# 10XGenomics/supernova

Measured on AMD Instinct MI355X. Metric: Gk-mers/s through count+graph at k=48, 1.2B×150bp; bit-exact counts, higher is better.
Workload: dtype u64

## Files before the change

supernova_amd/csrc/snk_count.hip:

```cpp
#include "snk_ctx.h"
#include "snk_common.h"
#include "snk_kernels.h"
#include "snk_stages.h"

namespace {

constexpr uint32_t BC_MULTI = 0xFFFFFFFEu;
constexpr uint32_t BC_IGN = 0xFFFFFFFFu;
static_assert(BC_IGN > BC_MULTI, "barcode states are merged with atomicMax");
#ifndef SNK_TIGHT_TRIES
#define SNK_TIGHT_TRIES 48
#endif
constexpr int MAX_SPLIT_LOG2 = 20;
#define SNK_COUNT_MAXSEG 32
#ifndef SNK_COUNT_THREADS
#define SNK_COUNT_THREADS 768
#endif
#ifndef SNK_SCREEN_ROUNDS
#define SNK_SCREEN_ROUNDS 6
#endif
#ifndef SNK_GSCREEN_SLOTS
#define SNK_GSCREEN_SLOTS 1024
#endif
#ifndef SNK_GSCREEN_BATCH
#define SNK_GSCREEN_BATCH 512
#endif
#ifndef SNK_GSCREEN_ROUNDS
#define SNK_GSCREEN_ROUNDS (SNK_SCREEN_ROUNDS + 4)
#endif
#ifndef SNK_NGSCREEN_PLANE_WORDS
#define SNK_NGSCREEN_PLANE_WORDS 512
#endif
#ifndef SNK_COUNT_SLOTS
#define SNK_COUNT_SLOTS 2048
#endif
#define LDS_LOAD(p) __hip_atomic_load((p), __ATOMIC_RELAXED, __HIP_MEMORY_SCOPE_WORKGROUP)
__device__ __forceinline__ void lds_barrier() { asm volatile("s_waitcnt lgkmcnt(0)\n\ts_barrier" ::: "memory"); }
#ifdef SNK_COUNT_PROF
#define PROF(n) do { if (tid == 0) { const long long _t = clock64(); prof_acc[n] += (unsigned long long)(_t - prof_t); prof_t = _t; } } while (0)
#else
#define PROF(n) do {} while (0)
#endif

__device__ __forceinline__ uint32_t funnel(uint32_t hi, uint32_t lo, uint32_t sh) {
#ifdef SNK_FUNNEL_ALIGNBIT
    return sh ? __builtin_amdgcn_alignbit(hi, lo, 32u - sh) : hi;
#else
    return (uint32_t)(((((uint64_t)hi << 32) | lo) << sh) >> 32);
#endif
}

template <int K> struct lo_t { typedef uint32_t type; };
template <> struct lo_t<60> { typedef uint64_t type; };

template <int K> __device__ __forceinline__ typename lo_t<K>::type lo_pack(uint64_t lo);
template <> __device__ __forceinline__ uint32_t lo_pack<48>(uint64_t lo) { return (uint32_t)(lo >> 32); }
template <> __device__ __forceinline__ uint64_t lo_pack<60>(uint64_t lo) { return lo; }
template <int K> __device__ __forceinline__ uint64_t lo_unpack(typename lo_t<K>::type v);
template <> __device__ __forceinline__ uint64_t lo_unpack<48>(uint32_t v) { return (uint64_t)v << 32; }
template <> __device__ __forceinline__ uint64_t lo_unpack<60>(uint64_t v) { return v; }

template <int K, bool G> struct klo_t { typedef typename lo_t<K>::type type; };
template <int K> struct klo_t<K, true> { typedef uint64_t type; };
template <int K, bool G> __device__ __forceinline__ typename klo_t<K, G>::type klo_pack(uint64_t lo) {
    if constexpr (G) return lo; else return lo_pack<K>(lo);
}
template <int K, bool G> __device__ __forceinline__ uint64_t klo_unpack(typename klo_t<K, G>::type v) {
    if constexpr (G) return v; else return lo_unpack<K>(v);
}

typedef __attribute__((address_space(3))) void* snk_lptr;

template <int K, int THREADS, int SLOTS, bool GROUPED, bool MULTI, bool GATHER = false, bool TIGHT = false, bool SCREEN = false>
__global__ void __launch_bounds__(THREADS, 6) snk_count_kernel(snk_count_args a) {
    constexpr int BATCH = (GROUPED && SCREEN && SLOTS <= 1024 && K == 48) ? SNK_GSCREEN_BATCH : ((K == 48 && !GROUPED && (SLOTS >= 2048 || SCREEN)) ? 512 : 256);
    constexpr int DD = 2 * BATCH;
    typedef typename klo_t<K, GROUPED>::type lo_type;
    constexpr int WMAX = K - SNK_M_MIN_OF(K) + 1;
    constexpr int NCI = BATCH * WMAX / 32 + 2;
    extern __shared__ __attribute__((aligned(16))) unsigned char smem_raw[];
    uint64_t* khi = reinterpret_cast<uint64_t*>(smem_raw);
    lo_type* klo = reinterpret_cast<lo_type*>(khi + SLOTS);
    uint32_t* tag = reinterpret_cast<uint32_t*>(klo + SLOTS);
    uint32_t* cnt = tag + SLOTS;
    uint32_t* bcs = cnt + SLOTS;
    uint32_t* ctxw = bcs + SLOTS;
    uint32_t* rec = ctxw + SLOTS / 4;
    uint32_t* ctl = rec + 8 * BATCH;
    uint32_t* dd = ctl + (TIGHT ? 72 : 64);
    uint32_t* wgt = dd + DD;
    uint16_t* lead = reinterpret_cast<uint16_t*>(wgt + BATCH);
    uint16_t* lpre = lead + BATCH;
    uint16_t* cidx = lpre + BATCH + 2;
    uint32_t* segi = reinterpret_cast<uint32_t*>(smem_raw + (((size_t)(reinterpret_cast<unsigned char*>(cidx + NCI) - smem_raw) + 15) & ~(size_t)15));
    uint16_t* olist = reinterpret_cast<uint16_t*>(segi + 2 * 3 * SNK_COUNT_MAXSEG);
    uint32_t* bcx = reinterpret_cast<uint32_t*>(smem_raw + (((size_t)(reinterpret_cast<unsigned char*>(olist + (TIGHT ? SLOTS - 64 : SLOTS - THREADS - 64)) - smem_raw) + 15) & ~(size_t)15));
    const bool bcset = a.bc_mode > 2;
    constexpr int SROUNDS = (SCREEN && SLOTS <= 1024) ? SNK_GSCREEN_ROUNDS : SNK_SCREEN_ROUNDS;
    static_assert(SROUNDS >= 1 && SROUNDS <= 16, "two cells per register");
    constexpr int SPW = GROUPED ? ((DD + BATCH) / 3 >= 512 ? 512 : 256) : SNK_NGSCREEN_PLANE_WORDS;
    constexpr uint32_t SCB = SPW == 1024 ? 17u : (SPW == 512 ? 18u : 19u);
    constexpr uint32_t SCAND = GROUPED ? (SLOTS <= 1024 ? 2048 : 1024) : 4096;
    uint16_t* cand = reinterpret_cast<uint16_t*>(bcx);
    uint32_t* planes = GROUPED ? dd : reinterpret_cast<uint32_t*>(cand + SCAND);
    static_assert(!SCREEN || (GROUPED && 3 * SPW <= DD + BATCH) || (!GROUPED && K == 48 && SLOTS <= 1024), "no room for the screen's bit planes");
    static_assert(THREADS >= BATCH && THREADS % 64 == 0, "the first BATCH threads own the staged records");
    const int tid = threadIdx.x;
    const int lane = tid & 63;
    const uint32_t LIMIT = TIGHT ? min(a.tight & 0xFFFFu, (uint32_t)SLOTS - 64u) : SLOTS - THREADS - 64;
    const int tight_tries = (int)(a.tight >> 16);
#ifdef SNK_COUNT_PROF
    long long prof_t = clock64();
    unsigned long long prof_acc[8] = {0, 0, 0, 0, 0, 0, 0, 0};
#endif
    auto dma_batch = [&](uint64_t base, uint64_t vend, const uint32_t* bnd, const uint32_t* seg) {
        constexpr int CH = 2 * BATCH;
        uint32_t seg_incl = 0;
        if (MULTI) {
            const uint32_t mylen = (uint32_t)lane < a.nseg ? LDS_LOAD(&seg[2 * SNK_COUNT_MAXSEG + lane]) - LDS_LOAD(&seg[lane]) : 0u;
            seg_incl = snk_wave_scan_incl(mylen);
        }
        constexpr int NR = (CH + THREADS - 1) / THREADS;
        uint32_t gx[NR];
        if (GATHER) {
#pragma unroll
            for (int r = 0; r < NR; ++r) {
                const int c = r * THREADS + tid;
                const uint64_t v = base + (uint32_t)(c >> 1);
                gx[r] = (c < CH && v < vend) ? a.gidx[v] : 0u;
            }
        }
#pragma unroll
        for (int r = 0; r * THREADS < CH; ++r) {
            const int c = r * THREADS + tid;
            const uint64_t v = base + (uint32_t)(c >> 1);
            if (c < CH && v < vend) {
                uint64_t gi;
                if (GATHER) gi = gx[r];
                else if (MULTI) {
                    const uint32_t x = (uint32_t)v;
                    uint32_t acc = 0, sg = 0;
                    for (uint32_t q = 0; q + 1 < a.nseg; ++q) { const uint32_t e = __builtin_amdgcn_readlane(seg_incl, q); if (x >= e) { sg = q + 1; acc = e; } }
                    gi = (((uint64_t)seg[SNK_COUNT_MAXSEG + sg] << 32) | seg[sg]) + (x - acc);
                } else gi = v;
                (void)bnd;
                const uint32_t lds_at = __builtin_amdgcn_readfirstlane((uint32_t)(size_t)(snk_lptr)(rec + 4 * (r * THREADS + (tid & ~63))));
                asm volatile("s_mov_b32 m0, %0\n\ts_nop 0\n\tglobal_load_lds_dwordx4 %1, off" :: "s"(lds_at), "v"(a.records + gi * 2 + (uint32_t)(c & 1)) : "memory");
            }
        }
    };
    auto bucket_range = [&](const uint32_t* bnd, const uint32_t* seg, uint64_t& vbeg, uint64_t& vend) {
        if (MULTI) {
            const uint32_t mylen = (uint32_t)lane < a.nseg ? LDS_LOAD(&seg[2 * SNK_COUNT_MAXSEG + lane]) - LDS_LOAD(&seg[lane]) : 0u;
            vbeg = 0;
            vend = (uint32_t)__builtin_amdgcn_readlane((int)snk_wave_scan_incl(mylen), 63);
        }
        else {
            vbeg = ((uint64_t)LDS_LOAD(&bnd[1]) << 32) | LDS_LOAD(&bnd[0]);
            vend = ((uint64_t)LDS_LOAD(&bnd[3]) << 32) | LDS_LOAD(&bnd[2]);
        }
    };
    const uint32_t G = a.bucket_stride;
    unsigned long long rcur = a.region_cursor[blockIdx.x];
    uint32_t bucket = a.bucket0 + (blockIdx.x + G - a.bucket0 % G) % G;
    uint32_t par = 0;
    {
        uint64_t b0 = 0, e0 = 0;
        if (tid == 0) {
            if (bucket < a.NB) { b0 = a.seg_beg[bucket]; e0 = a.seg_end[bucket]; }
            ctl[4] = (uint32_t)b0; ctl[5] = (uint32_t)(b0 >> 32); ctl[6] = (uint32_t)e0; ctl[7] = (uint32_t)(e0 >> 32);
            ctl[3] = 0;
            ctl[1] = 0; ctl[2] = 0; ctl[8] = 0; ctl[9] = 0; ctl[10] = 0; ctl[11] = 0; ctl[0] = 0;
            if (TIGHT) { ctl[64] = 0; ctl[65] = 0; }
        }
        for (int s = tid; s < SLOTS; s += THREADS) tag[s] = 0;
        if (MULTI && tid < (int)a.nseg) {
            uint64_t b = 0, e = 0;
            if (bucket < a.NB) { b = a.seg_beg[(uint64_t)tid * a.seg_stride + bucket]; e = a.seg_end[(uint64_t)tid * a.seg_stride + bucket]; }
            segi[tid] = (uint32_t)b; segi[SNK_COUNT_MAXSEG + tid] = (uint32_t)(b >> 32); segi[2 * SNK_COUNT_MAXSEG + tid] = (uint32_t)e;
        }
        lds_barrier();
        uint64_t vb, ve;
        bucket_range(ctl + 4, segi, vb, ve);
        dma_batch(vb, ve, ctl + 4, segi);
    }
    bool prefetched = true;
    uint32_t q = 0, bq = 0;
    unsigned long long claims_sum = 0;
    for (; bucket < a.NB; bucket += G) {
    uint32_t sp = 1;
    bool fresh = true;
    uint32_t splits_done = 0;
    const uint32_t nbucket = bucket + G;
    bool seg_pending = true;
    const uint32_t* bcur = ctl + 4 + 8 * par;
    uint32_t* bnext = ctl + 4 + 8 * (par ^ 1u);
    const uint32_t* segc = segi + par * (3 * SNK_COUNT_MAXSEG);
    uint32_t* segn = segi + (par ^ 1u) * (3 * SNK_COUNT_MAXSEG);
    const uint32_t sseg = MULTI ? min((uint32_t)tid, a.nseg - 1u) : 0u;
    auto load_next = [&](uint64_t& nbeg, uint64_t& nend, uint64_t& nsb, uint32_t& nse) {
        nbeg = 0; nend = 0; nsb = 0; nse = 0;
        if (nbucket < a.NB) {
            nbeg = a.seg_beg[nbucket]; nend = a.seg_end[nbucket];
            if (MULTI) { nsb = a.seg_beg[(uint64_t)sseg * a.seg_stride + nbucket]; nse = (uint32_t)a.seg_end[(uint64_t)sseg * a.seg_stride + nbucket]; }
        }
    };
    auto put_down = [&](uint64_t nbeg, uint64_t nend, uint64_t nsb, uint32_t nse) {
        bnext[0] = (uint32_t)nbeg; bnext[1] = (uint32_t)(nbeg >> 32); bnext[2] = (uint32_t)nend; bnext[3] = (uint32_t)(nend >> 32);
        if (MULTI) { segn[sseg] = (uint32_t)nsb; segn[SNK_COUNT_MAXSEG + sseg] = (uint32_t)(nsb >> 32); segn[2 * SNK_COUNT_MAXSEG + sseg] = nse; }
        seg_pending = false;
    };
    uint32_t lg0 = 0, id0 = 0, real_bucket = bucket;
    if (a.vmeta) {
        const uint2 vm = a.vmeta[bucket];
        real_bucket = __builtin_amdgcn_readfirstlane(vm.x);
        lg0 = __builtin_amdgcn_readfirstlane(vm.y >> 24);
        id0 = __builtin_amdgcn_readfirstlane(vm.y & 0xFFFFFFu);
    }
    while (sp) {
        PROF(0);
        --sp;
        uint32_t split_lg = lg0, split_id = id0;
        if (!fresh) {
            lds_barrier();
            split_lg = LDS_LOAD(&ctl[16 + 2 * sp]); split_id = LDS_LOAD(&ctl[17 + 2 * sp]);
        }
        fresh = false;
        const uint32_t split_mask = (1u << split_lg) - 1u;
        uint32_t* occ = ctl + 1 + q;
        uint32_t* place = ctl + 8 + q;
        uint32_t* resv = ctl + 64 + q;
        uint64_t vbeg, vend;
        bucket_range(bcur, segc, vbeg, vend);
        if (vbeg >= vend) {
            lds_barrier();
            if (tid == 0) { ctl[1 + (q ^ 1u)] = 0; ctl[8 + (q ^ 1u)] = 0; if (TIGHT) ctl[64 + (q ^ 1u)] = 0; }
            if (seg_pending) {
                uint64_t nbeg, nend, nsb; uint32_t nse;
                load_next(nbeg, nend, nsb, nse);
                put_down(nbeg, nend, nsb, nse);
            }
            lds_barrier();
        }
        PROF(1);
        {
            for (uint64_t base = vbeg; base < vend; base += BATCH) {
                if (!prefetched) dma_batch(base, vend, bcur, segc);
                prefetched = false;
                if (tid < BATCH) wgt[tid] = (SCREEN && GROUPED) ? 0u : 1u;
                if (SCREEN && !GROUPED) { for (int qq = tid; qq < 3 * SPW; qq += THREADS) planes[qq] = 0; }
                for (int q = tid; q < DD; q += THREADS) dd[q] = 0;
                asm volatile("s_waitcnt vmcnt(0)" ::: "memory");
                lds_barrier();
                PROF(2);
                if (tid == 0) { ctl[1 + (q ^ 1u)] = 0; ctl[8 + (q ^ 1u)] = 0; ctl[10 + (bq ^ 1u)] = 0; if (TIGHT) ctl[64 + (q ^ 1u)] = 0; if (SCREEN) ctl[0] = 0; }
                const bool fetch_next = seg_pending;
                uint64_t nbeg = 0, nend = 0, nsb = 0; uint32_t nse = 0;
                if (fetch_next) load_next(nbeg, nend, nsb, nse);
                uint32_t nkm = 0;
                if (tid < BATCH && base + tid < vend) {
                    const uint4 ra = *reinterpret_cast<const uint4*>(rec + 8 * tid), rb = *reinterpret_cast<const uint4*>(rec + 8 * tid + 4);
                    nkm = rb.z & 0x7Fu;
                    if (a.dbg == 5 && ((rb.z >> 7) & 3u) != 3u) nkm = 0;
                    if (!GROUPED && a.dbg != 4 && nkm) {
                        uint32_t h = (ra.x * 0x9E3779B1u) ^ snk_rotl32(ra.y * 0x85EBCA77u, 7) ^ (ra.z * 0xC2B2AE3Du) ^ snk_rotl32(ra.w * 0x27D4EB2Fu, 13)
                                   ^ (rb.x * 0x165667B1u) ^ snk_rotl32(rb.y * 0xcc9e2d51u, 19) ^ (rb.z * 0x1b873593u);
                        h ^= h >> 15; h *= 0x846ca68bu; h ^= h >> 13;
                        uint32_t s = h & (DD - 1);
                        for (;;) {
                            uint32_t v = LDS_LOAD(&dd[s]);
                            if (v == 0) {
                                v = atomicCAS(&dd[s], 0u, (uint32_t)tid + 1u);
                                if (v == 0) break;
                            }
                            const uint32_t L = v - 1u;
                            const uint4 la = *reinterpret_cast<const uint4*>(rec + 8 * L);
                            const uint32_t lb0 = rec[8 * L + 4], lb1 = rec[8 * L + 5], lb2 = rec[8 * L + 6];
                            bool same = ((la.x ^ ra.x) | (la.y ^ ra.y) | (la.z ^ ra.z) | (la.w ^ ra.w) | (lb0 ^ rb.x) | (lb1 ^ rb.y) | (lb2 ^ rb.z)) == 0;
                            if (GROUPED || bcset) same = same && LDS_LOAD(&rec[8 * L + 7]) == rb.w;
                            if (same) {
                                atomicAdd(&wgt[L], 1u);
                                const uint32_t mine = GROUPED ? 0u : rb.w;
                                if (mine >= BC_MULTI) atomicMax(&rec[8 * L + 7], mine);
                                else if (mine) {
                                    uint32_t ob = atomicCAS(&rec[8 * L + 7], 0u, mine);
                                    if (ob != 0 && ob != mine && ob < BC_MULTI) atomicMax(&rec[8 * L + 7], BC_MULTI);
                                }
                                nkm = 0;
                                break;
                            }
                            s = (s + 1) & (DD - 1);
                        }
                    }
                }
                const uint32_t sv = nkm | (nkm ? 0x10000u : 0u);
                uint32_t incl = sv;
                incl = snk_wave_scan_incl(incl);
// ... 90 lines not shown
                        const uint32_t m6 = rp[6], w7 = rp[7];
                        const uint32_t wt = (SCREEN && GROUPED) ? 1u : wgt[i];
                        const uint32_t n_i = m6 & 0x7Fu, hasL = (m6 >> 7) & 1u, hasR = (m6 >> 8) & 1u;
                        const uint32_t j = g + n_i - lend;
                        const uint32_t bst = GROUPED ? 0u : w7;
                        const uint32_t o = hasL + j;
                        const uint32_t wi = o >> 4, sh = (2u * o) & 31u;
                        const uint32_t* wp = rp + wi;
                        const uint32_t P = wp[-1], W0 = wp[0], W1 = wp[1], W2 = wp[2], W3 = wp[3];
                        const uint32_t F0 = funnel(W0, W1, sh), F1 = funnel(W1, W2, sh), F2 = funnel(W2, W3, sh);
                        const uint32_t pb = funnel(P, W0, sh) & 3u;
                        uint32_t F3 = 0, nb;
                        if constexpr (K == 48) nb = (W3 >> (30u - sh)) & 3u;
                        else {
                            static_assert(K == 60, "K is 48 or 60");
                            const uint32_t W4 = wp[4];
                            const uint32_t f3 = funnel(W3, W4, sh);
                            nb = (f3 >> 6) & 3u;
                            F3 = f3 & 0xFFFFFF00u;
                        }
                        const uint32_t havesucc = hasR | ((j + 1u - n_i) >> 31), havepred = min(o, 1u);
                        snk_kmer f;
                        f.hi = ((uint64_t)F0 << 32) | F1;
                        f.lo = ((uint64_t)F2 << 32) | F3;
                        const snk_kmer r = snk_kmer_rc<K>(f);
                        const bool rev = snk_kmer_lt(r, f);
                        snk_kmer c = rev ? r : f;
                        const uint32_t cfw = (havepred << (4u + pb)) | (havesucc << nb);
                        const uint32_t crv = (havesucc << (7u - nb)) | (havepred << (3u - pb));
                        const uint32_t ctx = rev ? crv : cfw;
                        if (GROUPED) c.lo |= (uint64_t)w7;
                        uint32_t h1, h2;
                        snk_kmer_hash_count<(K > 48) || GROUPED>(c, &h1, &h2);
                        if (a.dbg == 1) { if (h1 == 0x12345u && h2 == 0x54321u) a.status[3] = 7; }
                        else if ((h2 & split_mask) == split_id) {
                            uint32_t slot = h1 & (SLOTS - 1);
                            const uint32_t stride = ((h1 >> 16) ^ (h2 >> 20)) | 1u;
                            const lo_type clo = klo_pack<K, GROUPED>(c.lo);
                            const uint32_t mytag = (h2 & ~1u) | 2u;
                            bool claimed = false;
                            bool go = true;
                            uint32_t need = 0;
                            int rl = 0;
                            if constexpr (TIGHT) {
                                const unsigned long long pm = __ballot(1);
                                rl = __ffsll((long long)pm) - 1;
                                need = (uint32_t)__popcll(pm);
                                uint32_t r = 0;
                                if (lane == rl) {
                                    r = atomicAdd(resv, need);
                                    if ((r & 0x7FFFFFFFu) + need > LIMIT && !(r >> 31)) {
                                        atomicSub(resv, need);
                                        r = 0x80000000u;
                                        for (int tries = 0; tries < tight_tries; ++tries) {
                                            if (LDS_LOAD(occ) + need > LIMIT) break;
                                            const uint32_t rv = LDS_LOAD(resv);
                                            if (rv >> 31) break;
                                            if (rv + need <= LIMIT) {
                                                const uint32_t r2 = atomicAdd(resv, need);
                                                if (r2 >> 31) break;
                                                if (r2 + need <= LIMIT) { r = r2; break; }
                                                atomicSub(resv, need);
                                            }
                                            __builtin_amdgcn_s_sleep(2);
                                        }
                                        if (r >> 31) atomicOr(resv, 0x80000000u);
                                    }
                                }
                                go = (__shfl(r, rl) >> 31) == 0u;
                            }
                            if (go) {
                            for (;;) {
                                uint32_t t;
                                for (;;) {
                                    t = __hip_atomic_load(&tag[slot], __ATOMIC_ACQUIRE, __HIP_MEMORY_SCOPE_WORKGROUP);
                                    if (t == 0 || ((t ^ mytag) & ~1u) == 0) break;
                                    slot = (slot + stride) & (SLOTS - 1);
                                }
                                if (t == 0) {
                                    t = atomicCAS(&tag[slot], 0u, mytag);
                                    if (t == 0) {
                                        khi[slot] = c.hi;
                                        klo[slot] = clo;
                                        cnt[slot] = a.dbg == 2 ? 0u : wt;
                                        bcs[slot] = bst;
                                        reinterpret_cast<uint8_t*>(ctxw)[slot] = (uint8_t)ctx;
                                        if (bcset) {
#pragma unroll
                                            for (int q = 0; q < 6; ++q) bcx[slot * 6 + q] = 0;
                                        }
                                        __hip_atomic_store(&tag[slot], mytag | 1u, __ATOMIC_RELEASE, __HIP_MEMORY_SCOPE_WORKGROUP);
                                        claimed = true;
                                        break;
                                    }
                                    if (((t ^ mytag) & ~1u) != 0) { slot = (slot + stride) & (SLOTS - 1); continue; }
                                }
                                if (!(t & 1u)) continue;
                                if (khi[slot] == c.hi && klo[slot] == clo) break;
                                slot = (slot + stride) & (SLOTS - 1);
                            }
                            if constexpr (TIGHT) {
                                const uint32_t nc = (uint32_t)__popcll(__ballot(claimed));
                                if (lane == rl && need > nc) atomicSub(resv, need - nc);
                            }
                            if (claimed) {
                                const unsigned long long cm = __ballot(1);
                                const int leader = __ffsll((long long)cm) - 1;
                                uint32_t base = 0;
                                if (lane == leader) base = atomicAdd(occ, (uint32_t)__popcll(cm));
                                const uint32_t at = __shfl(base, leader) + (uint32_t)__popcll(cm & ((1ull << lane) - 1ull));
                                if (at < LIMIT) olist[at] = (uint16_t)slot;
                            } else if (a.dbg != 2) {
                                atomicAdd(&cnt[slot], wt);
                                if (ctx) atomicOr(&ctxw[slot >> 2], ctx << (8 * (slot & 3)));
                                if (bst >= BC_MULTI) atomicMax(&bcs[slot], bst);
                                else if (bst) {
                                    uint32_t ob = atomicCAS(&bcs[slot], 0u, bst);
                                    if (ob != 0 && ob != bst && ob < BC_MULTI) {
                                        if (!bcset) atomicMax(&bcs[slot], BC_MULTI);
                                        else {
                                            bool stored = false;
                                            for (int q = 0; q < 6 && !stored; ++q) {
                                                const uint32_t ov = atomicCAS(&bcx[slot * 6 + q], 0u, bst);
                                                stored = ov == 0u || ov == bst;
                                            }
                                            if (!stored) atomicMax(&bcs[slot], BC_MULTI);
                                        }
                                    }
                                }
                            }
                            }
                        }
                    }
                }
                lds_barrier();
                PROF(5);
                bq ^= 1u;
            }
        }
        if (TIGHT ? (LDS_LOAD(resv) >> 31) != 0u : LDS_LOAD(occ) > LIMIT) {
            if (split_lg >= MAX_SPLIT_LOG2) { if (tid == 0) atomicExch(&a.status[1], 1u); }
            else {
                if (tid == 0) {
                    ctl[16 + 2 * sp] = split_lg + 1; ctl[17 + 2 * sp] = split_id;
                    ctl[18 + 2 * sp] = split_lg + 1; ctl[19 + 2 * sp] = split_id | (1u << split_lg);
                }
                sp += 2;
            }
            for (int s = tid; s < SLOTS; s += THREADS) tag[s] = 0;
            ++splits_done;
            q ^= 1u;
            continue;
        }
        PROF(6);
        if (sp == 0) {
            uint64_t nvb, nve;
            bucket_range(bnext, segn, nvb, nve);
            dma_batch(nvb, nve, bnext, segn);
            prefetched = true;
        }
        const uint32_t nocc = LDS_LOAD(occ);
        const uint64_t rbase = rcur;
        const uint64_t gbase = (uint64_t)blockIdx.x * a.region_cap + rbase;
        for (uint32_t e0 = 0; e0 < nocc; e0 += THREADS) {
            const uint32_t e = e0 + tid;
            uint32_t s = 0, c = 0;
            bool ok = false;
            if (e < nocc) {
                s = olist[e];
                c = cnt[s];
                tag[s] = 0;
                ok = c >= a.min_freq && c != 0;
                if (ok && a.bc_mode) {
                    const uint32_t b = bcs[s];
                    if (!bcset) ok = a.bc_mode == 1 ? (b != 0) : (b >= BC_MULTI);
                    else {
                        uint32_t distinct = b ? 1u : 0u;
                        for (int j = 0; j < 6; ++j) distinct += bcx[s * 6 + j] ? 1u : 0u;
                        ok = b >= BC_MULTI || distinct >= a.bc_mode;
                    }
                }
            }
            const unsigned long long m = __ballot(ok);
            if (m) {
                const int leader = __ffsll((long long)m) - 1;
                uint32_t b = 0;
                if (lane == leader) b = atomicAdd(place, (uint32_t)__popcll(m));
                b = __builtin_amdgcn_readlane(b, leader);
                const uint64_t pos = rbase + b + (uint32_t)__popcll(m & ((1ull << lane) - 1ull));
                if (ok && pos < a.region_cap) {
                    const uint64_t at = gbase - rbase + pos;
                    const uint32_t cx = (ctxw[s >> 2] >> (8 * (s & 3))) & 0xFFu;
                    a.out_keys[at] = ((snk_u128)khi[s] << 64) | (snk_u128)klo_unpack<K, GROUPED>(klo[s]);
                    a.out_vals[at] = ((uint64_t)(c < 0xFFFFFFu ? c : 0xFFFFFFu) << 8) | cx;
                }
            }
        }
        lds_barrier();
        const uint32_t nvalid = LDS_LOAD(place);
        if constexpr (TIGHT) {
            if (a.chunk_n && nvalid > SNK_GRAPH_CHUNK_MAX && split_lg >= MAX_SPLIT_LOG2) { if (tid == 0) atomicExch(&a.status[1], 1u); }
            else if (a.chunk_n && nvalid > SNK_GRAPH_CHUNK_MAX) {
                if (tid == 0) {
                    ctl[16 + 2 * sp] = split_lg + 1; ctl[17 + 2 * sp] = split_id;
                    ctl[18 + 2 * sp] = split_lg + 1; ctl[19 + 2 * sp] = split_id | (1u << split_lg);
                }
                sp += 2;
                ++splits_done;
                asm volatile("s_waitcnt vmcnt(0)" ::: "memory");
                prefetched = false;
                q ^= 1u;
                continue;
            }
        }
        if (nvalid) {
            rcur += nvalid;
            if (tid == 0) {
                if (rbase + nvalid > a.region_cap) a.status[0] = 1;
                else if (a.chunk_n) {
                    if (split_lg == 0) { a.chunk_n[bucket] = nvalid; a.chunk_base[bucket] = (uint32_t)rbase; }
                    else {
                        const uint32_t e = atomicAdd(&a.status[4], 1u);
                        if (e < a.extra_cap) a.extra[e] = make_uint4(real_bucket, (uint32_t)rbase, nvalid | (blockIdx.x << 12), (split_lg << 24) | split_id);
                    }
                }
            }
        }
        claims_sum += nocc;
        if (tid == 0 && nocc > ctl[3]) ctl[3] = nocc;
        q ^= 1u;
        PROF(7);
    }
    if (tid == 0 && splits_done) atomicAdd(&a.status[2], 1u);
    par ^= 1u;
    }
    if (tid == 0) { a.region_cursor[blockIdx.x] = rcur; atomicMax(&a.status[3], ctl[3]); atomicAdd(&a.status[5], (uint32_t)(claims_sum >> 4)); }
    asm volatile("s_waitcnt vmcnt(0)" ::: "memory");
#ifdef SNK_COUNT_PROF
    if (tid == 0) for (int q = 0; q < 8; ++q) atomicAdd(&a.prof[q], prof_acc[q]);
#endif
}

template <int K> struct cfg;
template <> struct cfg<48> { static constexpr int THREADS = SNK_COUNT_THREADS; static constexpr int SLOTS = SNK_COUNT_SLOTS; };
template <> struct cfg<60> { static constexpr int THREADS = SNK_COUNT_THREADS; static constexpr int SLOTS = SNK_COUNT_SLOTS; };

template <int K, bool G>
size_t lds_bytes(uint32_t bc_mode = 0, bool tight = false, bool screen = false) {
    const size_t S = screen ? SNK_GSCREEN_SLOTS : cfg<K>::SLOTS, B = (G && screen && S <= 1024 && K == 48) ? SNK_GSCREEN_BATCH : ((K == 48 && !G && (S >= 2048 || screen)) ? 512 : 256), DD = 2 * B, NCI = B * (K - SNK_M_MIN_OF(K) + 1) / 32 + 2;
    return S * (8 + sizeof(typename klo_t<K, G>::type) + 4 + 4 + 4) + S + 4 * (8 * B + (tight ? 72 : 64) + DD + B) + 2 * (B + B + 2 + NCI) + 16 + 2 * 4 * 3 * SNK_COUNT_MAXSEG + 2 * (tight ? S - 64 : S - cfg<K>::THREADS - 64) + 16 + (bc_mode > 2 ? S * 24 + 16 : 0) + (screen ? (G ? (S <= 1024 ? 4096 : 2048) : 8192 + 3 * SNK_NGSCREEN_PLANE_WORDS * 4) + 16 : 0);
}

template <int K, bool G>
int launch(hipStream_t st, const snk_count_args& a, char* err, size_t errcap) {
    auto kern = a.nseg > 1 ? snk_count_kernel<K, cfg<K>::THREADS, cfg<K>::SLOTS, G, true> : snk_count_kernel<K, cfg<K>::THREADS, cfg<K>::SLOTS, G, false>;
    if (a.gidx) {
        if (a.nseg != 1) return snk_fail(SNK_E_INTERNAL, err, errcap, "count: an index list comes with one segment per bucket");
        kern = snk_count_kernel<K, cfg<K>::THREADS, cfg<K>::SLOTS, G, false, true>;
    }
    const bool tight = a.tight && !a.gidx;
    const bool screen = K == 48 && tight && a.screen >= 2u && a.bc_mode <= 2u;
    static_assert(SNK_GSCREEN_SLOTS <= 1024, "the ungrouped SCREEN instantiation needs the LDS half a table frees");
    if constexpr (K == 48) {
        if (screen) kern = a.nseg > 1 ? snk_count_kernel<K, cfg<K>::THREADS, SNK_GSCREEN_SLOTS, G, true, false, true, true> : snk_count_kernel<K, cfg<K>::THREADS, SNK_GSCREEN_SLOTS, G, false, false, true, true>;
    }
    if (tight && !screen) kern = a.nseg > 1 ? snk_count_kernel<K, cfg<K>::THREADS, cfg<K>::SLOTS, G, true, false, true> : snk_count_kernel<K, cfg<K>::THREADS, cfg<K>::SLOTS, G, false, false, true>;
    size_t lds = lds_bytes<K, G>(a.bc_mode, tight, screen);
    SNK_HIP_TRY(hipFuncSetAttribute((const void*)kern, hipFuncAttributeMaxDynamicSharedMemorySize, (int)lds));
    if (a.bucket0 >= a.NB) return SNK_OK;
    snk_count_args b = a;
    b.bucket_stride = a.n_regions;
    SNK_HIP_TRY(snk_launch(kern, a.n_regions, cfg<K>::THREADS, lds, st, b));
    return SNK_OK;
}

template <int K, bool G>
int regions(uint32_t nseg, uint32_t NB, uint32_t bc_mode, uint32_t persist, uint32_t* out, char* err, size_t errcap) {
    auto kern = nseg > 1 ? snk_count_kernel<K, cfg<K>::THREADS, cfg<K>::SLOTS, G, true> : snk_count_kernel<K, cfg<K>::THREADS, cfg<K>::SLOTS, G, false>;
    size_t lds = lds_bytes<K, G>(bc_mode);
    SNK_HIP_TRY(hipFuncSetAttribute((const void*)kern, hipFuncAttributeMaxDynamicSharedMemorySize, (int)lds));
    if (persist == 0) persist = 1;
    int per_cu = 0, dev = 0, n_cu = 256;
    SNK_HIP_TRY(hipOccupancyMaxActiveBlocksPerMultiprocessor(&per_cu, kern, cfg<K>::THREADS, lds));
    SNK_HIP_TRY(hipGetDevice(&dev));
    SNK_HIP_TRY(hipDeviceGetAttribute(&n_cu, hipDeviceAttributeMultiprocessorCount, dev));
    uint64_t grid = (uint64_t)(per_cu > 0 ? per_cu : 1) * (uint64_t)n_cu * persist;
    if (grid > NB) grid = NB;
    if (grid > (1u << 20)) grid = 1u << 20;
    *out = grid ? (uint32_t)grid : 1u;
    return SNK_OK;
}

}

namespace {
__global__ void __launch_bounds__(256) compact_regions_kernel(const snk_u128* __restrict__ keys_in, const uint64_t* __restrict__ vals_in,
                                                              uint64_t region_cap, const unsigned long long* __restrict__ cursor,
                                                              const unsigned long long* __restrict__ off,
                                                              snk_u128* __restrict__ keys_out, uint64_t* __restrict__ vals_out) {
    const uint32_t r = blockIdx.x;
    const uint64_t n = cursor[r], src = (uint64_t)r * region_cap, dst = off[r];
    for (uint64_t i = threadIdx.x; i < n; i += 256) {
        keys_out[dst + i] = keys_in[src + i];
        vals_out[dst + i] = vals_in[src + i];
    }
}
}

int snk_launch_compact_regions(hipStream_t st, const snk_u128* keys_in, const uint64_t* vals_in, uint64_t region_cap,
                               uint32_t n_regions, const unsigned long long* region_cursor,
                               const unsigned long long* region_off, snk_u128* keys_out, uint64_t* vals_out, char* err,
// ... 33 lines not shown
```

supernova_amd/csrc/snk_stages.hip:

```cpp
#include <string.h>
#include <cstring>
#include <rocprim/rocprim.hpp>

#include <stdlib.h>
#include <math.h>

#include <cmath>
#include <vector>

#include "snk_ctx.h"
#include "snk_common.h"
#include "snk_graph.h"
#include "snk_kernels.h"
#include "snk_stages.h"


int snk_stage_count_table(snk_ctx* ctx, hipStream_t st, uint32_t K, const void* records, const uint64_t* seg_beg,
                          const uint64_t* seg_end, uint32_t seg_stride, uint32_t nseg, uint32_t NB, uint32_t min_freq, uint32_t bc_mode, uint32_t grouped, uint64_t n_inst_hint,
                          uint32_t* status, bool want_sort, snk_table* out, char* err, size_t errcap, const snk_count_ranges* ranges, snk_count_pilot* pilot,
                          const uint32_t* gidx, bool defer_compact, const snk_hot* hot) {
    if (hot && hot->NBv == 0) hot = nullptr;
    defer_compact = defer_compact && !want_sort && snk_opt_u32(ctx, SNK_OPT_defer_compact) != 0;
    int rc;
    snk_phase_timer tm(st), kt(st);
// ... 162 lines not shown
            snk_count_args cv = ca;
            cv.records = (const uint4*)hot->records;
            cv.seg_beg = hot->seg;
            cv.seg_end = hot->seg + hot->NBv;
            cv.seg_stride = hot->NBv;
            cv.nseg = 1;
            cv.gidx = nullptr;
            cv.vmeta = hot->vmeta;
            cv.NB = hot->NBv;
            cv.bucket0 = 0;
            if ((rc = snk_launch_count(K, st, cv, err, errcap))) return rc;
        }
        if (pilot_regrow) {
            snk_ctx_release_block(ctx, keys_r);
            snk_ctx_release_block(ctx, vals_r);
            if (extra) snk_ctx_release_block(ctx, extra);
            pilot_regrown = true;
            --attempt;
            continue;
        }
        SNK_HIP_TRY(hipMemcpyAsync(h_rcur.data(), rcur, n_regions * 8ull, hipMemcpyDeviceToHost, st));
        SNK_HIP_TRY(hipMemcpyAsync(h_status, status, 32, hipMemcpyDeviceToHost, st));
        SNK_HIP_TRY(snk_sync(st));
#ifdef SNK_COUNT_PROF
        {
            unsigned long long hp[8];
            (void)hipMemcpy(hp, ca.prof, 64, hipMemcpyDeviceToHost);
            unsigned long long tot = 0;
            for (int q = 0; q < 8; ++q) tot += hp[q];
            fprintf(stderr, "[snk prof] count kernel, cycles of thread 0 per phase (%% of total): control %.1f, clear %.1f, stage %.1f, dedupe+scan %.1f, map %.1f, insert %.1f, emit-count %.1f, emit-write %.1f\n",
                    100.0 * hp[0] / tot, 100.0 * hp[1] / tot, 100.0 * hp[2] / tot, 100.0 * hp[3] / tot, 100.0 * hp[4] / tot, 100.0 * hp[5] / tot, 100.0 * hp[6] / tot, 100.0 * hp[7] / tot);
        }
#endif
        if (ca.dbg >= 2) {
            unsigned long long d[3];
            (void)hipMemcpy(d, status + 4, 24, hipMemcpyDeviceToHost);
            fprintf(stderr, "[snk dbg] lane probe iterations %llu, wave-level iterations %llu, max lane iterations in one probe %llu\n", d[0], d[1], d[2]);
        }
        if (h_status[1]) return snk_fail(SNK_E_INTERNAL, err, errcap, h_status[1] == 2 ? "count: a table probe did not terminate" : "count: bucket split depth exceeded");
        unsigned long long mx = 0;
        n_kmers = 0;
        for (uint32_t r = 0; r < n_regions; ++r) { n_kmers += h_rcur[r]; if (h_rcur[r] > mx) mx = h_rcur[r]; }
        const bool extra_ovf = !want_sort && h_status[4] > extra_cap;
        if (!h_status[0] && mx <= region_cap && !extra_ovf) break;
        if (attempt == 3) return snk_fail(SNK_E_INTERNAL, err, errcap, "count: region overflow (%llu > %llu)", mx, (unsigned long long)region_cap);
        snk_ctx_release_block(ctx, keys_r);
        snk_ctx_release_block(ctx, vals_r);
        if (mx > region_cap) region_cap = mx + 64;
        if (extra_ovf) extra_cap = h_status[4] + 64;
    }
    if (ranges && ranges->finished) ranges->finished(ranges->user);
    {
        std::vector<unsigned long long>& h_off = ctx->h_region_off;
        h_off.resize(n_regions + 1);
        unsigned long long acc = 0;
        for (uint32_t r = 0; r < n_regions; ++r) { h_off[r] = acc; acc += h_rcur[r]; }
        h_off[n_regions] = acc;
        SNK_HIP_TRY(hipMemcpyAsync(roff, h_off.data(), (n_regions + 1) * 8ull, hipMemcpyHostToDevice, st));
        void* q;
        if ((rc = snk_ctx_alloc(ctx, (n_kmers + 1) * 16, &q, err, errcap))) return rc; keys_a = (snk_u128*)q;
        if ((rc = snk_ctx_alloc(ctx, (n_kmers + 1) * 8, &q, err, errcap))) return rc; vals_a = (uint64_t*)q;
        out->keys_r = nullptr; out->vals_r = nullptr; out->region_cap = region_cap;
        if (defer_compact) {
            snk_ctx_release_block(ctx, vals_a);
            vals_a = nullptr;
            out->keys_r = keys_r; out->vals_r = vals_r;
        } else {
            if ((rc = snk_launch_compact_regions(st, keys_r, vals_r, region_cap, n_regions, rcur, roff, keys_a, vals_a, err, errcap))) return rc;
            snk_ctx_release_block(ctx, keys_r);
            snk_ctx_release_block(ctx, vals_r);
        }
// ... 764 lines not shown
```

Measured before the change: 98.21.

## Cut count-kernel SGPR pressure: cold kernarg loads, templated barcode mode, multi-segment fast path

Result: faster. 99.80 (median of 6 runs) (+1.6%).

```diff
diff --git a/supernova_amd/csrc/snk_count.hip b/supernova_amd/csrc/snk_count.hip
--- a/supernova_amd/csrc/snk_count.hip
+++ b/supernova_amd/csrc/snk_count.hip
@@ -50,6 +50,13 @@
 #endif
 }
 
+typedef const __attribute__((address_space(4))) snk_count_args* count_kargs_t;
+__device__ __forceinline__ count_kargs_t cold_args() {
+    count_kargs_t p = (count_kargs_t)__builtin_amdgcn_kernarg_segment_ptr();
+    asm volatile("" : "+s"(p));
+    return p;
+}
+
 template <int K> struct lo_t { typedef uint32_t type; };
 template <> struct lo_t<60> { typedef uint64_t type; };
 
@@ -71,7 +78,7 @@
 
 typedef __attribute__((address_space(3))) void* snk_lptr;
 
-template <int K, int THREADS, int SLOTS, bool GROUPED, bool MULTI, bool GATHER = false, bool TIGHT = false, bool SCREEN = false>
+template <int K, int THREADS, int SLOTS, bool GROUPED, bool MULTI, bool GATHER = false, bool TIGHT = false, bool SCREEN = false, bool BCSET = false>
 __global__ void __launch_bounds__(THREADS, 6) snk_count_kernel(snk_count_args a) {
     constexpr int BATCH = (GROUPED && SCREEN && SLOTS <= 1024 && K == 48) ? SNK_GSCREEN_BATCH : ((K == 48 && !GROUPED && (SLOTS >= 2048 || SCREEN)) ? 512 : 256);
     constexpr int DD = 2 * BATCH;
@@ -93,9 +100,16 @@
     uint16_t* lpre = lead + BATCH;
     uint16_t* cidx = lpre + BATCH + 2;
     uint32_t* segi = reinterpret_cast<uint32_t*>(smem_raw + (((size_t)(reinterpret_cast<unsigned char*>(cidx + NCI) - smem_raw) + 15) & ~(size_t)15));
-    uint16_t* olist = reinterpret_cast<uint16_t*>(segi + 2 * 3 * SNK_COUNT_MAXSEG);
+    uint32_t* mseg = segi + 2 * 3 * SNK_COUNT_MAXSEG;
+    uint16_t* olist = reinterpret_cast<uint16_t*>(mseg + 4);
     uint32_t* bcx = reinterpret_cast<uint32_t*>(smem_raw + (((size_t)(reinterpret_cast<unsigned char*>(olist + (TIGHT ? SLOTS - 64 : SLOTS - THREADS - 64)) - smem_raw) + 15) & ~(size_t)15));
-    const bool bcset = a.bc_mode > 2;
+    constexpr bool bcset = BCSET;
+    static_assert(!BCSET || (!GROUPED && !SCREEN), "grouped runs have no barcode rule, SCREEN keeps at most two barcodes per slot");
+#ifdef SNK_PROBES
+    const uint32_t dbg = a.dbg;
+#else
+    constexpr uint32_t dbg = 0;
+#endif
     constexpr int SROUNDS = (SCREEN && SLOTS <= 1024) ? SNK_GSCREEN_ROUNDS : SNK_SCREEN_ROUNDS;
     static_assert(SROUNDS >= 1 && SROUNDS <= 16, "two cells per register");
     constexpr int SPW = GROUPED ? ((DD + BATCH) / 3 >= 512 ? 512 : 256) : SNK_NGSCREEN_PLANE_WORDS;
@@ -113,10 +127,10 @@
     long long prof_t = clock64();
     unsigned long long prof_acc[8] = {0, 0, 0, 0, 0, 0, 0, 0};
 #endif
-    auto dma_batch = [&](uint64_t base, uint64_t vend, const uint32_t* bnd, const uint32_t* seg) {
+    auto dma_batch = [&](uint64_t base, uint64_t vend, const uint32_t* seg, bool multi) {
         constexpr int CH = 2 * BATCH;
         uint32_t seg_incl = 0;
-        if (MULTI) {
+        if (MULTI && multi) {
             const uint32_t mylen = (uint32_t)lane < a.nseg ? LDS_LOAD(&seg[2 * SNK_COUNT_MAXSEG + lane]) - LDS_LOAD(&seg[lane]) : 0u;
             seg_incl = snk_wave_scan_incl(mylen);
         }
@@ -137,20 +151,20 @@
             if (c < CH && v < vend) {
                 uint64_t gi;
                 if (GATHER) gi = gx[r];
-                else if (MULTI) {
+                else if (MULTI && multi) {
                     const uint32_t x = (uint32_t)v;
                     uint32_t acc = 0, sg = 0;
                     for (uint32_t q = 0; q + 1 < a.nseg; ++q) { const uint32_t e = __builtin_amdgcn_readlane(seg_incl, q); if (x >= e) { sg = q + 1; acc = e; } }
                     gi = (((uint64_t)seg[SNK_COUNT_MAXSEG + sg] << 32) | seg[sg]) + (x - acc);
                 } else gi = v;
-                (void)bnd;
                 const uint32_t lds_at = __builtin_amdgcn_readfirstlane((uint32_t)(size_t)(snk_lptr)(rec + 4 * (r * THREADS + (tid & ~63))));
                 asm volatile("s_mov_b32 m0, %0\n\ts_nop 0\n\tglobal_load_lds_dwordx4 %1, off" :: "s"(lds_at), "v"(a.records + gi * 2 + (uint32_t)(c & 1)) : "memory");
             }
         }
     };
-    auto bucket_range = [&](const uint32_t* bnd, const uint32_t* seg, uint64_t& vbeg, uint64_t& vend) {
-        if (MULTI) {
+    auto bucket_range = [&](const uint32_t* bnd, const uint32_t* seg, const uint32_t* more, uint64_t& vbeg, uint64_t& vend) -> bool {
+        const bool multi = MULTI && __builtin_amdgcn_readfirstlane(LDS_LOAD(more)) != 0u;
+        if (multi) {
             const uint32_t mylen = (uint32_t)lane < a.nseg ? LDS_LOAD(&seg[2 * SNK_COUNT_MAXSEG + lane]) - LDS_LOAD(&seg[lane]) : 0u;
             vbeg = 0;
             vend = (uint32_t)__builtin_amdgcn_readlane((int)snk_wave_scan_incl(mylen), 63);
@@ -159,6 +173,7 @@
             vbeg = ((uint64_t)LDS_LOAD(&bnd[1]) << 32) | LDS_LOAD(&bnd[0]);
             vend = ((uint64_t)LDS_LOAD(&bnd[3]) << 32) | LDS_LOAD(&bnd[2]);
         }
+        return multi;
     };
     const uint32_t G = a.bucket_stride;
     unsigned long long rcur = a.region_cursor[blockIdx.x];
@@ -174,15 +189,19 @@
             if (TIGHT) { ctl[64] = 0; ctl[65] = 0; }
         }
         for (int s = tid; s < SLOTS; s += THREADS) tag[s] = 0;
-        if (MULTI && tid < (int)a.nseg) {
+        if (MULTI) {
             uint64_t b = 0, e = 0;
-            if (bucket < a.NB) { b = a.seg_beg[(uint64_t)tid * a.seg_stride + bucket]; e = a.seg_end[(uint64_t)tid * a.seg_stride + bucket]; }
-            segi[tid] = (uint32_t)b; segi[SNK_COUNT_MAXSEG + tid] = (uint32_t)(b >> 32); segi[2 * SNK_COUNT_MAXSEG + tid] = (uint32_t)e;
+            if (tid < (int)a.nseg) {
+                if (bucket < a.NB) { b = a.seg_beg[(uint64_t)tid * a.seg_stride + bucket]; e = a.seg_end[(uint64_t)tid * a.seg_stride + bucket]; }
+                segi[tid] = (uint32_t)b; segi[SNK_COUNT_MAXSEG + tid] = (uint32_t)(b >> 32); segi[2 * SNK_COUNT_MAXSEG + tid] = (uint32_t)e;
+            }
+            const unsigned long long mm = __ballot(tid >= 1 && tid < (int)a.nseg && (uint32_t)e != (uint32_t)b);
+            if (tid == 0) mseg[0] = mm != 0ull;
         }
         lds_barrier();
         uint64_t vb, ve;
-        bucket_range(ctl + 4, segi, vb, ve);
-        dma_batch(vb, ve, ctl + 4, segi);
+        const bool m0 = bucket_range(ctl + 4, segi, mseg, vb, ve);
+        dma_batch(vb, ve, segi, m0);
     }
     bool prefetched = true;
     uint32_t q = 0, bq = 0;
@@ -201,18 +220,24 @@
     auto load_next = [&](uint64_t& nbeg, uint64_t& nend, uint64_t& nsb, uint32_t& nse) {
         nbeg = 0; nend = 0; nsb = 0; nse = 0;
         if (nbucket < a.NB) {
-            nbeg = a.seg_beg[nbucket]; nend = a.seg_end[nbucket];
-            if (MULTI) { nsb = a.seg_beg[(uint64_t)sseg * a.seg_stride + nbucket]; nse = (uint32_t)a.seg_end[(uint64_t)sseg * a.seg_stride + nbucket]; }
+            const count_kargs_t ka = cold_args();
+            const uint64_t* sb = ka->seg_beg; const uint64_t* se = ka->seg_end;
+            nbeg = sb[nbucket]; nend = se[nbucket];
+            if (MULTI) { const uint64_t at = (uint64_t)sseg * ka->seg_stride + nbucket; nsb = sb[at]; nse = (uint32_t)se[at]; }
         }
     };
     auto put_down = [&](uint64_t nbeg, uint64_t nend, uint64_t nsb, uint32_t nse) {
         bnext[0] = (uint32_t)nbeg; bnext[1] = (uint32_t)(nbeg >> 32); bnext[2] = (uint32_t)nend; bnext[3] = (uint32_t)(nend >> 32);
-        if (MULTI) { segn[sseg] = (uint32_t)nsb; segn[SNK_COUNT_MAXSEG + sseg] = (uint32_t)(nsb >> 32); segn[2 * SNK_COUNT_MAXSEG + sseg] = nse; }
+        if (MULTI) {
+            segn[sseg] = (uint32_t)nsb; segn[SNK_COUNT_MAXSEG + sseg] = (uint32_t)(nsb >> 32); segn[2 * SNK_COUNT_MAXSEG + sseg] = nse;
+            const unsigned long long mm = __ballot(tid >= 1 && tid < (int)a.nseg && nse != (uint32_t)nsb);
+            if (tid == 0) mseg[par ^ 1u] = mm != 0ull;
+        }
         seg_pending = false;
     };
     uint32_t lg0 = 0, id0 = 0, real_bucket = bucket;
-    if (a.vmeta) {
-        const uint2 vm = a.vmeta[bucket];
+    if (const uint2* vmeta = cold_args()->vmeta) {
+        const uint2 vm = vmeta[bucket];
         real_bucket = __builtin_amdgcn_readfirstlane(vm.x);
         lg0 = __builtin_amdgcn_readfirstlane(vm.y >> 24);
         id0 = __builtin_amdgcn_readfirstlane(vm.y & 0xFFFFFFu);
@@ -231,7 +256,7 @@
         uint32_t* place = ctl + 8 + q;
         uint32_t* resv = ctl + 64 + q;
         uint64_t vbeg, vend;
-        bucket_range(bcur, segc, vbeg, vend);
+        const bool mcur = bucket_range(bcur, segc, mseg + par, vbeg, vend);
         if (vbeg >= vend) {
             lds_barrier();
             if (tid == 0) { ctl[1 + (q ^ 1u)] = 0; ctl[8 + (q ^ 1u)] = 0; if (TIGHT) ctl[64 + (q ^ 1u)] = 0; }
@@ -245,7 +270,7 @@
         PROF(1);
         {
             for (uint64_t base = vbeg; base < vend; base += BATCH) {
-                if (!prefetched) dma_batch(base, vend, bcur, segc);
+                if (!prefetched) dma_batch(base, vend, segc, mcur);
                 prefetched = false;
                 if (tid < BATCH) wgt[tid] = (SCREEN && GROUPED) ? 0u : 1u;
                 if (SCREEN && !GROUPED) { for (int qq = tid; qq < 3 * SPW; qq += THREADS) planes[qq] = 0; }
@@ -261,8 +286,8 @@
                 if (tid < BATCH && base + tid < vend) {
                     const uint4 ra = *reinterpret_cast<const uint4*>(rec + 8 * tid), rb = *reinterpret_cast<const uint4*>(rec + 8 * tid + 4);
                     nkm = rb.z & 0x7Fu;
-                    if (a.dbg == 5 && ((rb.z >> 7) & 3u) != 3u) nkm = 0;
-                    if (!GROUPED && a.dbg != 4 && nkm) {
+                    if (dbg == 5 && ((rb.z >> 7) & 3u) != 3u) nkm = 0;
+                    if (!GROUPED && dbg != 4 && nkm) {
                         uint32_t h = (ra.x * 0x9E3779B1u) ^ snk_rotl32(ra.y * 0x85EBCA77u, 7) ^ (ra.z * 0xC2B2AE3Du) ^ snk_rotl32(ra.w * 0x27D4EB2Fu, 13)
                                    ^ (rb.x * 0x165667B1u) ^ snk_rotl32(rb.y * 0xcc9e2d51u, 19) ^ (rb.z * 0x1b873593u);
                         h ^= h >> 15; h *= 0x846ca68bu; h ^= h >> 13;
@@ -419,7 +444,7 @@
                         if (GROUPED) c.lo |= (uint64_t)w7;
                         uint32_t h1, h2;
                         snk_kmer_hash_count<(K > 48) || GROUPED>(c, &h1, &h2);
-                        if (a.dbg == 1) { if (h1 == 0x12345u && h2 == 0x54321u) a.status[3] = 7; }
+                        if (dbg == 1) { if (h1 == 0x12345u && h2 == 0x54321u) cold_args()->status[3] = 7; }
                         else if ((h2 & split_mask) == split_id) {
                             uint32_t slot = h1 & (SLOTS - 1);
                             const uint32_t stride = ((h1 >> 16) ^ (h2 >> 20)) | 1u;
@@ -469,7 +494,7 @@
                                     if (t == 0) {
                                         khi[slot] = c.hi;
                                         klo[slot] = clo;
-                                        cnt[slot] = a.dbg == 2 ? 0u : wt;
+                                        cnt[slot] = dbg == 2 ? 0u : wt;
                                         bcs[slot] = bst;
                                         reinterpret_cast<uint8_t*>(ctxw)[slot] = (uint8_t)ctx;
                                         if (bcset) {
@@ -497,7 +522,7 @@
                                 if (lane == leader) base = atomicAdd(occ, (uint32_t)__popcll(cm));
                                 const uint32_t at = __shfl(base, leader) + (uint32_t)__popcll(cm & ((1ull << lane) - 1ull));
                                 if (at < LIMIT) olist[at] = (uint16_t)slot;
-                            } else if (a.dbg != 2) {
+                            } else if (dbg != 2) {
                                 atomicAdd(&cnt[slot], wt);
                                 if (ctx) atomicOr(&ctxw[slot >> 2], ctx << (8 * (slot & 3)));
                                 if (bst >= BC_MULTI) atomicMax(&bcs[slot], bst);
@@ -526,7 +551,7 @@
             }
         }
         if (TIGHT ? (LDS_LOAD(resv) >> 31) != 0u : LDS_LOAD(occ) > LIMIT) {
-            if (split_lg >= MAX_SPLIT_LOG2) { if (tid == 0) atomicExch(&a.status[1], 1u); }
+            if (split_lg >= MAX_SPLIT_LOG2) { if (tid == 0) atomicExch(&cold_args()->status[1], 1u); }
             else {
                 if (tid == 0) {
                     ctl[16 + 2 * sp] = split_lg + 1; ctl[17 + 2 * sp] = split_id;
@@ -542,13 +567,18 @@
         PROF(6);
         if (sp == 0) {
             uint64_t nvb, nve;
-            bucket_range(bnext, segn, nvb, nve);
-            dma_batch(nvb, nve, bnext, segn);
+            const bool mnext = bucket_range(bnext, segn, mseg + (par ^ 1u), nvb, nve);
+            dma_batch(nvb, nve, segn, mnext);
             prefetched = true;
         }
         const uint32_t nocc = LDS_LOAD(occ);
         const uint64_t rbase = rcur;
-        const uint64_t gbase = (uint64_t)blockIdx.x * a.region_cap + rbase;
+        const count_kargs_t ka = cold_args();
+        const uint64_t region_cap = ka->region_cap;
+        snk_u128* const out_keys = ka->out_keys;
+        uint64_t* const out_vals = ka->out_vals;
+        const uint32_t min_freq = ka->min_freq, bc_mode = ka->bc_mode;
+        const uint64_t gbase = (uint64_t)blockIdx.x * region_cap + rbase;
         for (uint32_t e0 = 0; e0 < nocc; e0 += THREADS) {
             const uint32_t e = e0 + tid;
             uint32_t s = 0, c = 0;
@@ -557,14 +587,14 @@
                 s = olist[e];
                 c = cnt[s];
                 tag[s] = 0;
-                ok = c >= a.min_freq && c != 0;
-                if (ok && a.bc_mode) {
+                ok = c >= min_freq && c != 0;
+                if (ok && bc_mode) {
                     const uint32_t b = bcs[s];
-                    if (!bcset) ok = a.bc_mode == 1 ? (b != 0) : (b >= BC_MULTI);
+                    if (!bcset) ok = bc_mode == 1 ? (b != 0) : (b >= BC_MULTI);
                     else {
                         uint32_t distinct = b ? 1u : 0u;
                         for (int j = 0; j < 6; ++j) distinct += bcx[s * 6 + j] ? 1u : 0u;
-                        ok = b >= BC_MULTI || distinct >= a.bc_mode;
+                        ok = b >= BC_MULTI || distinct >= bc_mode;
                     }
                 }
             }
@@ -575,19 +605,20 @@
                 if (lane == leader) b = atomicAdd(place, (uint32_t)__popcll(m));
                 b = __builtin_amdgcn_readlane(b, leader);
                 const uint64_t pos = rbase + b + (uint32_t)__popcll(m & ((1ull << lane) - 1ull));
-                if (ok && pos < a.region_cap) {
+                if (ok && pos < region_cap) {
                     const uint64_t at = gbase - rbase + pos;
                     const uint32_t cx = (ctxw[s >> 2] >> (8 * (s & 3))) & 0xFFu;
-                    a.out_keys[at] = ((snk_u128)khi[s] << 64) | (snk_u128)klo_unpack<K, GROUPED>(klo[s]);
-                    a.out_vals[at] = ((uint64_t)(c < 0xFFFFFFu ? c : 0xFFFFFFu) << 8) | cx;
+                    out_keys[at] = ((snk_u128)khi[s] << 64) | (snk_u128)klo_unpack<K, GROUPED>(klo[s]);
+                    out_vals[at] = ((uint64_t)(c < 0xFFFFFFu ? c : 0xFFFFFFu) << 8) | cx;
                 }
             }
         }
         lds_barrier();
         const uint32_t nvalid = LDS_LOAD(place);
         if constexpr (TIGHT) {
-            if (a.chunk_n && nvalid > SNK_GRAPH_CHUNK_MAX && split_lg >= MAX_SPLIT_LOG2) { if (tid == 0) atomicExch(&a.status[1], 1u); }
-            else if (a.chunk_n && nvalid > SNK_GRAPH_CHUNK_MAX) {
+            const bool chunked = nvalid > SNK_GRAPH_CHUNK_MAX && cold_args()->chunk_n != nullptr;
+            if (chunked && split_lg >= MAX_SPLIT_LOG2) { if (tid == 0) atomicExch(&cold_args()->status[1], 1u); }
+            else if (chunked) {
                 if (tid == 0) {
                     ctl[16 + 2 * sp] = split_lg + 1; ctl[17 + 2 * sp] = split_id;
                     ctl[18 + 2 * sp] = split_lg + 1; ctl[19 + 2 * sp] = split_id | (1u << split_lg);
@@ -603,12 +634,13 @@
         if (nvalid) {
             rcur += nvalid;
             if (tid == 0) {
-                if (rbase + nvalid > a.region_cap) a.status[0] = 1;
-                else if (a.chunk_n) {
-                    if (split_lg == 0) { a.chunk_n[bucket] = nvalid; a.chunk_base[bucket] = (uint32_t)rbase; }
+                const count_kargs_t kc = cold_args();
+                if (rbase + nvalid > kc->region_cap) kc->status[0] = 1;
+                else if (uint32_t* const chunk_n = kc->chunk_n) {
+                    if (split_lg == 0) { chunk_n[bucket] = nvalid; kc->chunk_base[bucket] = (uint32_t)rbase; }
                     else {
-                        const uint32_t e = atomicAdd(&a.status[4], 1u);
-                        if (e < a.extra_cap) a.extra[e] = make_uint4(real_bucket, (uint32_t)rbase, nvalid | (blockIdx.x << 12), (split_lg << 24) | split_id);
+                        const uint32_t e = atomicAdd(&kc->status[4], 1u);
+                        if (e < kc->extra_cap) kc->extra[e] = make_uint4(real_bucket, (uint32_t)rbase, nvalid | (blockIdx.x << 12), (split_lg << 24) | split_id);
                     }
                 }
             }
@@ -621,10 +653,10 @@
     if (tid == 0 && splits_done) atomicAdd(&a.status[2], 1u);
     par ^= 1u;
     }
-    if (tid == 0) { a.region_cursor[blockIdx.x] = rcur; atomicMax(&a.status[3], ctl[3]); atomicAdd(&a.status[5], (uint32_t)(claims_sum >> 4)); }
+    if (tid == 0) { const count_kargs_t kc = cold_args(); kc->region_cursor[blockIdx.x] = rcur; atomicMax(&kc->status[3], ctl[3]); atomicAdd(&kc->status[5], (uint32_t)(claims_sum >> 4)); }
     asm volatile("s_waitcnt vmcnt(0)" ::: "memory");
 #ifdef SNK_COUNT_PROF
-    if (tid == 0) for (int q = 0; q < 8; ++q) atomicAdd(&a.prof[q], prof_acc[q]);
+    if (tid == 0) for (int q = 0; q < 8; ++q) atomicAdd(&cold_args()->prof[q], prof_acc[q]);
 #endif
 }
 
@@ -635,23 +667,33 @@
 template <int K, bool G>
 size_t lds_bytes(uint32_t bc_mode = 0, bool tight = false, bool screen = false) {
     const size_t S = screen ? SNK_GSCREEN_SLOTS : cfg<K>::SLOTS, B = (G && screen && S <= 1024 && K == 48) ? SNK_GSCREEN_BATCH : ((K == 48 && !G && (S >= 2048 || screen)) ? 512 : 256), DD = 2 * B, NCI = B * (K - SNK_M_MIN_OF(K) + 1) / 32 + 2;
-    return S * (8 + sizeof(typename klo_t<K, G>::type) + 4 + 4 + 4) + S + 4 * (8 * B + (tight ? 72 : 64) + DD + B) + 2 * (B + B + 2 + NCI) + 16 + 2 * 4 * 3 * SNK_COUNT_MAXSEG + 2 * (tight ? S - 64 : S - cfg<K>::THREADS - 64) + 16 + (bc_mode > 2 ? S * 24 + 16 : 0) + (screen ? (G ? (S <= 1024 ? 4096 : 2048) : 8192 + 3 * SNK_NGSCREEN_PLANE_WORDS * 4) + 16 : 0);
+    return S * (8 + sizeof(typename klo_t<K, G>::type) + 4 + 4 + 4) + S + 4 * (8 * B + (tight ? 72 : 64) + DD + B) + 2 * (B + B + 2 + NCI) + 16 + 2 * 4 * 3 * SNK_COUNT_MAXSEG + 16 + 2 * (tight ? S - 64 : S - cfg<K>::THREADS - 64) + 16 + (bc_mode > 2 ? S * 24 + 16 : 0) + (screen ? (G ? (S <= 1024 ? 4096 : 2048) : 8192 + 3 * SNK_NGSCREEN_PLANE_WORDS * 4) + 16 : 0);
+}
+
+typedef void (*count_kernel_t)(snk_count_args);
+template <int K, bool G, bool BC>
+count_kernel_t plain_kernel(bool multi, bool gather, bool tight) {
+    constexpr int T = cfg<K>::THREADS, S = cfg<K>::SLOTS;
+    if (gather) return snk_count_kernel<K, T, S, G, false, true, false, false, BC>;
+    if (tight) return multi ? snk_count_kernel<K, T, S, G, true, false, true, false, BC> : snk_count_kernel<K, T, S, G, false, false, true, false, BC>;
+    return multi ? snk_count_kernel<K, T, S, G, true, false, false, false, BC> : snk_count_kernel<K, T, S, G, false, false, false, false, BC>;
+}
+template <int K, bool G>
+count_kernel_t plain_kernel(uint32_t bc_mode, bool multi, bool gather, bool tight) {
+    if constexpr (!G) { if (bc_mode > 2) return plain_kernel<K, G, true>(multi, gather, tight); }
+    return plain_kernel<K, G, false>(multi, gather, tight);
 }
 
 template <int K, bool G>
 int launch(hipStream_t st, const snk_count_args& a, char* err, size_t errcap) {
-    auto kern = a.nseg > 1 ? snk_count_kernel<K, cfg<K>::THREADS, cfg<K>::SLOTS, G, true> : snk_count_kernel<K, cfg<K>::THREADS, cfg<K>::SLOTS, G, false>;
-    if (a.gidx) {
-        if (a.nseg != 1) return snk_fail(SNK_E_INTERNAL, err, errcap, "count: an index list comes with one segment per bucket");
-        kern = snk_count_kernel<K, cfg<K>::THREADS, cfg<K>::SLOTS, G, false, true>;
-    }
+    if (a.gidx && a.nseg != 1) return snk_fail(SNK_E_INTERNAL, err, errcap, "count: an index list comes with one segment per bucket");
     const bool tight = a.tight && !a.gidx;
     const bool screen = K == 48 && tight && a.screen >= 2u && a.bc_mode <= 2u;
     static_assert(SNK_GSCREEN_SLOTS <= 1024, "the ungrouped SCREEN instantiation needs the LDS half a table frees");
+    count_kernel_t kern = plain_kernel<K, G>(a.bc_mode, a.nseg > 1, a.gidx != nullptr, tight);
     if constexpr (K == 48) {
         if (screen) kern = a.nseg > 1 ? snk_count_kernel<K, cfg<K>::THREADS, SNK_GSCREEN_SLOTS, G, true, false, true, true> : snk_count_kernel<K, cfg<K>::THREADS, SNK_GSCREEN_SLOTS, G, false, false, true, true>;
     }
-    if (tight && !screen) kern = a.nseg > 1 ? snk_count_kernel<K, cfg<K>::THREADS, cfg<K>::SLOTS, G, true, false, true> : snk_count_kernel<K, cfg<K>::THREADS, cfg<K>::SLOTS, G, false, false, true>;
     size_t lds = lds_bytes<K, G>(a.bc_mode, tight, screen);
     SNK_HIP_TRY(hipFuncSetAttribute((const void*)kern, hipFuncAttributeMaxDynamicSharedMemorySize, (int)lds));
     if (a.bucket0 >= a.NB) return SNK_OK;
@@ -663,7 +705,7 @@
 
 template <int K, bool G>
 int regions(uint32_t nseg, uint32_t NB, uint32_t bc_mode, uint32_t persist, uint32_t* out, char* err, size_t errcap) {
-    auto kern = nseg > 1 ? snk_count_kernel<K, cfg<K>::THREADS, cfg<K>::SLOTS, G, true> : snk_count_kernel<K, cfg<K>::THREADS, cfg<K>::SLOTS, G, false>;
+    count_kernel_t kern = plain_kernel<K, G>(bc_mode, nseg > 1, false, false);
     size_t lds = lds_bytes<K, G>(bc_mode);
     SNK_HIP_TRY(hipFuncSetAttribute((const void*)kern, hipFuncAttributeMaxDynamicSharedMemorySize, (int)lds));
     if (persist == 0) persist = 1;
diff --git a/supernova_amd/csrc/snk_stages.hip b/supernova_amd/csrc/snk_stages.hip
--- a/supernova_amd/csrc/snk_stages.hip
+++ b/supernova_amd/csrc/snk_stages.hip
@@ -218,11 +218,13 @@
                     100.0 * hp[0] / tot, 100.0 * hp[1] / tot, 100.0 * hp[2] / tot, 100.0 * hp[3] / tot, 100.0 * hp[4] / tot, 100.0 * hp[5] / tot, 100.0 * hp[6] / tot, 100.0 * hp[7] / tot);
         }
 #endif
+#ifdef SNK_PROBES
         if (ca.dbg >= 2) {
             unsigned long long d[3];
             (void)hipMemcpy(d, status + 4, 24, hipMemcpyDeviceToHost);
             fprintf(stderr, "[snk dbg] lane probe iterations %llu, wave-level iterations %llu, max lane iterations in one probe %llu\n", d[0], d[1], d[2]);
         }
+#endif
         if (h_status[1]) return snk_fail(SNK_E_INTERNAL, err, errcap, h_status[1] == 2 ? "count: a table probe did not terminate" : "count: bucket split depth exceeded");
         unsigned long long mx = 0;
         n_kmers = 0;
```
